# nianticlabs/simplerecon

Measured on AMD Instinct MI355X. Metric: depth frames/sec (640x480, 7 src views, 64 planes), higher is better.
Workload: dtype f32

## Files before the change

include/simplerecon_hip.h:

```cpp
#ifndef SIMPLERECON_HIP_H_
#define SIMPLERECON_HIP_H_

#include <stddef.h>
#include <stdint.h>

#ifdef __cplusplus
extern "C" {
#endif

#define SR_OK 0
#define SR_ERR_INVALID_ARGUMENT 1
#define SR_ERR_UNSUPPORTED 2
#define SR_ERR_WORKSPACE_TOO_SMALL 3
#define SR_ERR_HIP_BASE 1000

enum {
  SR_OPT_MLP_SPLIT = 0, SR_OPT_WINO_SPLIT, SR_OPT_WINO_XCD, SR_OPT_WINO_NT, SR_OPT_WINO_KSPLIT, SR_OPT_CONV_WINO,
  SR_OPT_CONV_TILE, SR_OPT_CONV_KSPLIT, SR_OPT_PW_NT, SR_OPT_PW_KS, SR_OPT_PT_CFG, SR_OPT_PT_KS, SR_OPT_DOT_LDS,
  SR_OPT_DOT_LDS_G, SR_OPT_DOT_LDS_CULL, SR_OPT_DOT_LDS_CAP, SR_OPT_UPSAMPLE_QUAD, SR_OPT_POOL_STREAM,
  SR_OPT_COUNT
};
int sr_option_count(void);
const char* sr_option_name(int id);
int sr_option_id(const char* name);
int sr_option_get(int id, int* value);
int sr_option_set(int id, int value, int* previous );
int sr_option_default(int id, int* value);

int sr_abi_version(void);

const char* sr_target_arch(void);


size_t sr_volume_workspace_bytes(int B, int K, int C, int h, int w);

int sr_volume_prepare(const float* src, const float* K_src, const float* T_src_cur,
                      const float* T_cur_src, int B, int K, int C, int h, int w, void* workspace,
                      size_t workspace_bytes, void* stream);

int sr_dot_volume_sweep(const float* cur, const float* invK_cur, const float* planes, int64_t ps_b,
                        int64_t ps_d, int64_t ps_y, int64_t ps_x, int B, int K, int C, int h, int w,
                        int D, float* out_cv, int64_t cv_sb, int64_t cv_sd, int64_t cv_sp,
                        float* out_lowest, uint8_t* out_mask, void* workspace,
                        size_t workspace_bytes, void* stream);

int sr_conv3x3_wino_io_nhwc_fwd(const void* in, int64_t in_batch_stride, int in_pix_stride, const float* packed_u,
                                const float* bias, const void* residual, int64_t res_batch_stride, int res_pix_stride,
                                void* out, int64_t out_batch_stride, int out_pix_stride, int B, int H, int W, int Cin,
                                int Cout, float leaky_slope, int io_dtype, void* stream);
int sr_pw_conv_io_nhwc_fwd(const void* in, int64_t in_batch_stride, int in_pix_stride, const float* packed_w,
                           const float* bias, const void* residual, int64_t res_batch_stride, int res_pix_stride, void* out,
                           int64_t out_batch_stride, int out_pix_stride, int B, int HW, int Cin, int Cout, float act_code,
                           int io_dtype, void* stream);

size_t sr_pw_conv_tiled_workspace_bytes(int M, int Cin, int Cout);
int sr_pw_conv_tiled_plan(int M, int Cin, int Cout, int can_split, int* cfg, int* ks);
int sr_pw_conv_tiled_nhwc_fwd(const float* in, int in_pix_stride, const float* packed_w, const float* bias,
                              const float* gate, const float* residual, int res_pix_stride, float* out,
                              int out_pix_stride, int M, int HW, int Cin, int Cout, float act_code, void* workspace,
                              size_t workspace_bytes, void* stream);
int sr_pw_conv_supported(int Cin, int Cout);
int sr_pw_conv_plan(int B, int HW, int Cin, int Cout, int* nt, int* ks);
int sr_pw_conv_nhwc_fwd(const float* in, int64_t in_batch_stride, int in_pix_stride, const float* packed_w,
                        const float* bias, const float* gate, const float* residual, int64_t res_batch_stride,
                        int res_pix_stride, float* out, int64_t out_batch_stride, int out_pix_stride, int B, int HW,
                        int Cin, int Cout, float act_code, void* stream);

int sr_backproject_fwd(const float* depth, const float* invK, float* out_points, int B, int h, int w, void* stream);
int sr_project3d_fwd(const float* points, const float* K, const float* T, float* out, int B, int N, float eps,
                     void* stream);
int sr_backproject_bwd(const float* grad_points, const float* invK, float* grad_depth, int B, int h, int w, void* stream);
int sr_project3d_bwd(const float* grad_out, const float* points, const float* K, const float* T, float* grad_points, int B,
// ... 89 lines not shown

int sr_conv3x3_wino4_variant_nhwc_fwd(const float* in, int64_t in_batch_stride, int in_pix_stride, const float* packed_u,
                                      const float* bias, const float* residual, int64_t res_batch_stride,
                                      int res_pix_stride, float* out, int64_t out_batch_stride, int out_pix_stride, int B,
                                      int H, int W, int Cin, int Cout, float leaky_slope, int variant, void* stream);

int sr_wino_splitk_factor(int B, int H, int W, int Cin, int Cout);
size_t sr_wino_splitk_workspace_bytes(int B, int H, int W, int Cin, int Cout);
int sr_conv3x3_wino_splitk_nhwc_fwd(const float* in, int64_t in_batch_stride, int in_pix_stride,
                                    const float* packed_u, const float* bias, const float* residual,
                                    int64_t res_batch_stride, int res_pix_stride, float* out,
                                    int64_t out_batch_stride, int out_pix_stride, int B, int H, int W, int Cin,
                                    int Cout, float leaky_slope, void* workspace, size_t workspace_bytes,
                                    void* stream);

const char* sr_wino_kernel_name(int B, int H, int W, int Cin, int Cout, int aligned_in, int aligned_out);

const char* sr_conv_kernel_name(int B, int H, int W, int Cin, int Cout, int ksize, int stride, int aligned16);

int sr_upsample2x_nhwc_fwd(const float* in, int64_t in_batch_stride, int in_pix_stride, float* out,
                           int64_t out_batch_stride, int out_pix_stride, int B, int H, int W, int C,
                           void* stream);

int sr_exp_fwd(const float* in, float* out, int64_t n, void* stream);


size_t sr_stem_packed_weight_floats(int Cout);
int sr_stem_pack_weights(const float* weight, int Cout, float* packed, void* stream);

int sr_stem7x7_fwd(const float* in, int64_t in_batch_stride, int64_t in_chan_stride, int64_t in_row_stride,
                   int64_t in_col_stride, const float* packed_weight, const float* scale, const float* shift,
                   float leaky_slope, float* out, int64_t out_batch_stride, int out_pix_stride, int B, int H, int W,
                   int Cout, void* stream);

int sr_maxblurpool_nhwc_fwd(const float* in, int64_t in_batch_stride, int in_pix_stride, float* out,
                            int64_t out_batch_stride, int out_pix_stride, int B, int H, int W, int C, void* stream);

size_t sr_instance_norm_workspace_bytes(int B, int H, int W, int C);
int sr_instance_norm_nhwc_fwd(const float* in, int64_t in_batch_stride, int in_pix_stride, float* out,
                              int64_t out_batch_stride, int out_pix_stride, int B, int H, int W, int C, float eps,
                              float leaky_slope, void* workspace, size_t workspace_bytes, void* stream);

int sr_instance_norm_stats_nhwc(const float* in, int64_t in_batch_stride, int in_pix_stride, int B, int H, int W, int C,
                                float eps, float* stats, void* workspace, size_t workspace_bytes, void* stream);

size_t sr_conv1x1_stats_workspace_bytes(int B, int H, int W, int Cout);
int sr_conv1x1_stats_nhwc_fwd(const float* in, int64_t in_batch_stride, int in_pix_stride, const float* weight,
                              const float* bias, float* out, int64_t out_batch_stride, int out_pix_stride, int B, int H,
                              int W, int Cin, int Cout, float eps, float* stats, void* workspace, size_t workspace_bytes,
                              void* stream);

size_t sr_conv3x3_c16_packed_weight_floats(int Cout, int Cin);
int sr_conv3x3_c16_pack_weights(const float* weight, int Cout, int Cin, float* packed, void* stream);
int sr_conv3x3_c16_nhwc_fwd(const float* in, int64_t in_batch_stride, int in_pix_stride, const float* in_stats,
                            float in_leaky_slope, const float* packed_weight, const float* bias, float* out,
                            int64_t out_batch_stride, int out_pix_stride, int B, int H, int W, int Cin, int Cout,
                            int replicate, float leaky_slope, void* stream);

int sr_tsdf_integrate_fwd(void* tsdf_values, void* tsdf_weights, const void* voxel_coords, int X, int Y, int Z,
                          float origin_x, float origin_y, float origin_z, float voxel_size, const void* depth,
                          const uint8_t* depth_mask, const void* K, const void* T, int B, int H, int W,
                          float min_depth, float max_depth, float depth_range, float truncation, float maxW,
                          void* stream);

size_t sr_mesh_count_scratch_bytes(int X, int Y, int Z);
size_t sr_mesh_list_scratch_bytes(int64_t active);
int sr_mesh_count(const void* tsdf_values, int X, int Y, int Z, float level, void* count_scratch,
                  size_t count_scratch_bytes, int64_t* totals, void* stream);
int sr_mesh_emit(const void* tsdf_values, int X, int Y, int Z, float level, float origin_x, float origin_y, float origin_z,
                 float scale, const void* count_scratch, size_t count_scratch_bytes, void* list_scratch,
                 size_t list_scratch_bytes, int64_t active, int64_t num_vertices, int64_t num_faces, float* vertices,
                 float* normals, int* faces, void* stream);

#define SR_PC_FRAME_FLOATS 36
int sr_pc_consistency(const float* depth, const float* frame_consts, int N, int h, int w, int ref_begin, int ref_count,
                      float z_thresh, float* points, int* counts, void* stream);
int sr_pc_voxel_keys(const float* points, int64_t M, double min_x, double min_y, double min_z, double voxel_size,
                     int64_t* keys, void* stream);
int sr_pc_voxel_mean(const float* points, const uint8_t* colors, int64_t M, const int64_t* order,
                     const int64_t* seg_start, int64_t S, float* out_points, uint8_t* out_colors, void* stream);

#define SR_LOSS_MAX_SOURCES 15
size_t sr_normals_workspace_bytes(int B, int h, int w);
int sr_normals_fwd(const float* depth, const float* invK, int B, int h, int w, float* normals, void* scratch,
                   size_t scratch_bytes, void* stream);
int sr_normals_bwd(const float* grad_normals, const float* depth, const float* invK, int B, int h, int w,
                   float* grad_depth, void* scratch, size_t scratch_bytes, void* stream);
size_t sr_normals_loss_workspace_bytes(int B, int h, int w);
int sr_normals_loss_fwd(const float* normals_gt, const float* normals_pred, int B, int h, int w, float* out,
                        void* scratch, size_t scratch_bytes, void* stream);
int sr_normals_loss_bwd(const float* grad_out, const float* stats, const float* normals_gt, const float* normals_pred,
                        int B, int h, int w, float* grad_pred, void* stream);
size_t sr_grad_loss_workspace_bytes(int B, int h, int w);
int sr_grad_loss_fwd(const float* depth_gt, const float* depth_pred, int B, int h, int w, float* out, void* scratch,
                     size_t scratch_bytes, void* stream);
int sr_grad_loss_bwd(const float* grad_out, const float* stats, const float* depth_gt, const float* depth_pred, int B,
                     int h, int w, float* grad_pred, void* scratch, size_t scratch_bytes, void* stream);
size_t sr_mv_loss_workspace_bytes(int B, int K, int h, int w);
int sr_mv_loss_fwd(const float* depth_pred, const float* depth_gt, const float* src_depth, const float* cur_invK,
                   const float* src_K, const float* cur_world_T_cam, const float* src_cam_T_world, int B, int K, int h,
                   int w, float eps, float* out, uint8_t* valid_mask, float* sampled, void* scratch,
                   size_t scratch_bytes, void* stream);
int sr_mv_loss_bwd(const float* grad_out, const float* stats, const float* depth_pred, const float* depth_gt,
                   const float* src_depth, const float* cur_invK, const float* src_K, const float* cur_world_T_cam,
                   const float* src_cam_T_world, int B, int K, int h, int w, float eps, float* grad_pred,
                   void* stream);
// ... 221 lines not shown
```

simplerecon_amd/_lib.py:

```python
import contextlib
import ctypes as C
import os

import torch

_HERE = os.path.dirname(os.path.abspath(__file__))
LIB_PATH = os.environ.get("SR_HIP_LIBRARY") or os.path.join(_HERE, "libsimplerecon_hip.so")
ABI_VERSION = 3

_lib = None

_p = C.c_void_p
_i = C.c_int
_i64 = C.c_int64
_f = C.c_float
_sz = C.c_size_t

SIGNATURES = {
    "sr_abi_version": (_i, []),
    "sr_option_count": (_i, []),
    "sr_option_name": (C.c_char_p, [_i]),
    "sr_option_id": (_i, [C.c_char_p]),
    "sr_option_get": (_i, [_i, C.POINTER(C.c_int)]),
    "sr_option_set": (_i, [_i, _i, C.POINTER(C.c_int)]),
# ... 65 lines not shown
    "sr_norm_stats_nhwc": (_i, [_p, _i64, _i, _i, _i, _i, _i, _p, _p, _p, _sz, _p]),
    "sr_norm_act_fwd_nhwc": (_i, [_p, _i64, _i, _p, _p, _f, _p, _p, _f, _i, _p, _i64, _i, _i, _i, _i, _p]),
    "sr_norm_act_bwd_nhwc": (_i, [_p, _i64, _i, _p, _i64, _i, _p, _p, _f, _p, _p, _f, _i, _i, _p, _i64, _i, _p, _p,
                                  _i, _i, _i, _p, _sz, _p]),
    "sr_rowsum_nhwc": (_i, [_p, _i64, _i, _p, _i64, _i, _i, _i, _i, _f, _p, _p, _sz, _p]),
    "sr_maxblurpool_bwd_workspace_bytes": (_sz, [_i, _i, _i, _i]),
    "sr_maxblurpool_bwd_nhwc": (_i, [_p, _i64, _i, _p, _i64, _i, _p, _i64, _i, _i, _i, _i, _i, _p, _sz, _p]),
    "sr_replicate_pad_nhwc_fwd": (_i, [_p, _i64, _i, _p, _i, _i, _i, _i, _i, _p]),
    "sr_replicate_pad_nhwc_bwd": (_i, [_p, _p, _i, _i, _i, _i, _i, _p]),
    "sr_im2col7x7s2_nhwc": (_i, [_p, _i64, _i64, _i64, _i64, _p, _i, _i, _i, _i, _p]),
    "sr_dwconv3x3_bwd_workspace_bytes": (_sz, [_i, _i, _i, _i]),
    "sr_dwconv3x3_bwd_nhwc": (_i, [_p, _i64, _i, _p, _i64, _i, _p, _p, _p, _i, _i, _i, _i, _i, _i, _i, _i, _i, _p, _sz,
                                   _p]),
    "sr_scale_bwd_nhwc": (_i, [_p, _i64, _i, _p, _p, _f, _p, _i, _i, _i, _p]),
    "sr_small_linear_fwd": (_i, [_p, _p, _p, _p, _p, _i, _i, _i, _f, _p]),
    "sr_small_linear_bwd": (_i, [_p, _p, _p, _p, _p, _p, _p, _i, _i, _i, _f, _p]),
    "sr_act_in_bwd": (_i, [_p, _p, _p, _i64, _f, _p]),
    "sr_add_act_fwd": (_i, [_p, _p, _p, _p, _i64, _f, _p]),
    "sr_conv_wgrad_padded_workspace_bytes": (_sz, [_i, _i, _i, _i, _i, _i]),
    "sr_conv_wgrad_padded_nhwc": (_i, [_p, _i64, _i, _p, _i64, _i, _p, _i, _i, _i, _i, _i, _i, _i, _i, _i, _i, _i, _p,
                                       _sz, _p]),
    "sr_conv_splitk_workspace_bytes": (_sz, [_i, _i, _i, _i, _i, _i, _i]),
    "sr_conv2d_splitk_nhwc_fwd": (_i, [_p, _i64, _i, _p, _p, _p, _i64, _i, _p, _i64, _i, _i, _i, _i, _i, _i, _i, _i,
                                       _f, _p, _sz, _p]),
    "sr_wino_packed_weight_floats": (_sz, [_i, _i]),
    "sr_wino_pack_weights": (_i, [_p, _i, _i, _p, _p]),
    "sr_conv_prefers_wino": (_i, [_i, _i, _i, _i, _i, _i, _i]),
    "sr_wino_splitk_factor": (_i, [_i, _i, _i, _i, _i]),
    "sr_wino_splitk_workspace_bytes": (_sz, [_i, _i, _i, _i, _i]),
    "sr_conv3x3_wino_splitk_nhwc_fwd": (_i, [_p, _i64, _i, _p, _p, _p, _i64, _i, _p, _i64, _i, _i, _i, _i, _i, _i, _f,
                                             _p, _sz, _p]),
    "sr_wino_kernel_name": (C.c_char_p, [_i, _i, _i, _i, _i, _i, _i]),
    "sr_conv3x3_wino_nhwc_fwd": (_i, [_p, _i64, _i, _p, _p, _p, _i64, _i, _p, _i64, _i, _i, _i, _i, _i, _i, _f, _p]),
    "sr_wino4_packed_weight_floats": (_sz, [_i, _i]),
    "sr_wino4_pack_weights": (_i, [_p, _i, _i, _p, _p]),
    "sr_conv_prefers_wino4": (_i, [_i, _i, _i, _i, _i, _i]),
    "sr_conv3x3_wino4_nhwc_fwd": (_i, [_p, _i64, _i, _p, _p, _p, _i64, _i, _p, _i64, _i, _i, _i, _i, _i, _i, _f, _p]),
    "sr_conv3x3_wino4_variant_nhwc_fwd": (_i, [_p, _i64, _i, _p, _p, _p, _i64, _i, _p, _i64, _i, _i, _i, _i, _i, _i, _f, _i,
                                               _p]),
    "sr_conv_kernel_name": (C.c_char_p, [_i, _i, _i, _i, _i, _i, _i, _i]),
    "sr_upsample2x_nhwc_fwd": (_i, [_p, _i64, _i, _p, _i64, _i, _i, _i, _i, _i, _p]),
    "sr_exp_fwd": (_i, [_p, _p, _i64, _p]),
    "sr_stem_packed_weight_floats": (_sz, [_i]),
    "sr_stem_pack_weights": (_i, [_p, _i, _p, _p]),
    "sr_stem7x7_fwd": (_i, [_p, _i64, _i64, _i64, _i64, _p, _p, _p, _f, _p, _i64, _i, _i, _i, _i, _i, _p]),
    "sr_maxblurpool_nhwc_fwd": (_i, [_p, _i64, _i, _p, _i64, _i, _i, _i, _i, _i, _p]),
    "sr_instance_norm_workspace_bytes": (_sz, [_i, _i, _i, _i]),
    "sr_instance_norm_nhwc_fwd": (_i, [_p, _i64, _i, _p, _i64, _i, _i, _i, _i, _i, _f, _f, _p, _sz, _p]),
    "sr_instance_norm_stats_nhwc": (_i, [_p, _i64, _i, _i, _i, _i, _i, _f, _p, _p, _sz, _p]),
    "sr_conv1x1_stats_workspace_bytes": (_sz, [_i, _i, _i, _i]),
    "sr_conv1x1_stats_nhwc_fwd": (_i, [_p, _i64, _i, _p, _p, _p, _i64, _i, _i, _i, _i, _i, _i, _f, _p, _p, _sz, _p]),
    "sr_conv3x3_c16_packed_weight_floats": (_sz, [_i, _i]),
    "sr_conv3x3_c16_pack_weights": (_i, [_p, _i, _i, _p, _p]),
    "sr_conv3x3_c16_nhwc_fwd": (_i, [_p, _i64, _i, _p, _f, _p, _p, _p, _i64, _i, _i, _i, _i, _i, _i, _i, _f, _p]),
    "sr_tsdf_integrate_fwd": (_i, [_p, _p, _p, _i, _i, _i, _f, _f, _f, _f, _p, _p, _p, _p, _i, _i, _i,
                                   _f, _f, _f, _f, _f, _p]),
    "sr_mesh_count_scratch_bytes": (_sz, [_i, _i, _i]),
    "sr_mesh_list_scratch_bytes": (_sz, [_i64]),
    "sr_mesh_count": (_i, [_p, _i, _i, _i, _f, _p, _sz, _p, _p]),
    "sr_mesh_emit": (_i, [_p, _i, _i, _i, _f, _f, _f, _f, _f, _p, _sz, _p, _sz, _i64, _i64, _i64, _p, _p, _p, _p]),
    "sr_pc_consistency": (_i, [_p, _p, _i, _i, _i, _i, _i, _f, _p, _p, _p]),
    "sr_pc_voxel_keys": (_i, [_p, _i64, C.c_double, C.c_double, C.c_double, C.c_double, _p, _p]),
    "sr_pc_voxel_mean": (_i, [_p, _p, _i64, _p, _p, _i64, _p, _p, _p]),
    "sr_normals_workspace_bytes": (_sz, [_i, _i, _i]),
    "sr_normals_fwd": (_i, [_p, _p, _i, _i, _i, _p, _p, _sz, _p]),
    "sr_normals_bwd": (_i, [_p, _p, _p, _i, _i, _i, _p, _p, _sz, _p]),
    "sr_normals_loss_workspace_bytes": (_sz, [_i, _i, _i]),
    "sr_normals_loss_fwd": (_i, [_p, _p, _i, _i, _i, _p, _p, _sz, _p]),
    "sr_normals_loss_bwd": (_i, [_p, _p, _p, _p, _i, _i, _i, _p, _p]),
    "sr_grad_loss_workspace_bytes": (_sz, [_i, _i, _i]),
    "sr_grad_loss_fwd": (_i, [_p, _p, _i, _i, _i, _p, _p, _sz, _p]),
    "sr_grad_loss_bwd": (_i, [_p, _p, _p, _p, _i, _i, _i, _p, _p, _sz, _p]),
    "sr_mv_loss_workspace_bytes": (_sz, [_i, _i, _i, _i]),
    "sr_mv_loss_fwd": (_i, [_p, _p, _p, _p, _p, _p, _p, _i, _i, _i, _i, _f, _p, _p, _p, _p, _sz, _p]),
    "sr_mv_loss_bwd": (_i, [_p, _p, _p, _p, _p, _p, _p, _p, _p, _i, _i, _i, _i, _f, _p, _p]),
    "sr_depth_terms_workspace_bytes": (_sz, [_i, _i, _i]),
    "sr_depth_terms_fwd": (_i, [_p, _p, _p, _p, _p, _i, _i, _p, _i, _i, _p, _i, _i, _i, _i, _i, _f, _i, _p, _p, _sz,
                                _p]),
    "sr_depth_terms_bwd": (_i, [_p, _p, _p, _p, _p, _p, _p, _i, _i, _p, _i, _i, _p, _i, _i, _i, _i, _i, _f, _i, _p, _p,
                                _p, _p, _p, _p]),
    "sr_depth_metrics_workspace_bytes": (_sz, [_i, _i, _i]),
    "sr_depth_metrics": (_i, [_p, _p, _p, _f, _i, _i, _i, _i, _i, _i, _i, _p, _p, _p, _p, _sz, _p]),
    "sr_depth_metrics_gather": (_i, [_p, _i, _i, _i, _i, _i, _i, _p, _p]),
    "sr_nn_grid_plan": (_i, [_i64, _p, _i64, _p, _p, _p]),
    "sr_nn_keys": (_i, [_p, _i64, C.c_double, C.c_double, C.c_double, C.c_double, _i, _i, _i, _p, _p]),
    "sr_nn_build": (_i, [_p, _i64, _p, _p, _i64, _p, _p, _p]),
    "sr_nn_query": (_i, [_p, _i64, _p, _p, _i64, _p, _i64, C.c_double, C.c_double, C.c_double, C.c_double, _i, _i, _i,
                         _p, _p, _p, _p]),
    "sr_sample_surface_workspace_bytes": (_sz, [_i64]),
    "sr_sample_surface_cdf": (_i, [_p, _i64, _p, _i64, _p, _p, _sz, _p]),
    "sr_sample_surface": (_i, [_p, _i64, _p, _i64, _p, _i64, C.c_uint64, _p, _p, _p]),
    "sr_mesh_metrics_workspace_bytes": (_sz, [_i64, _i64]),
    "sr_mesh_metrics": (_i, [_p, _i64, _p, _i64, _f, _p, _p, _sz, _p]),
    "sr_stsdf_touch": (_i, [_p, _i, _i, _i, _p, C.c_double, C.c_double, _p, _p]),
    "sr_stsdf_block_masks": (_i, [_p, _p, _i64, _i64, _p, _p]),
    "sr_stsdf_integrate": (_i, [_p, _i64, _p, _p, _p, _i64, _p, _p, _p, _i, _i, _i, _f, _f, _p]),
    "sr_stsdf_mesh_count": (_i, [_p, _i64, _p, _p, _i64, _p, _p]),
    "sr_stsdf_mesh_emit": (_i, [_p, _i64, _p, _p, _i64, _f, _p, _i64, _i64, _p, _p, _p, _p, _p]),
    "sr_raster_small": (_i, [_p, _i64, _p, _i64, _p, _p, _i, _i, _i, _f, _f, _i, _p, _p, _p]),
    "sr_raster_large_setup": (_i, [_p, _i64, _p, _i64, _p, _p, _i, _i, _i, _f, _f, _i, _i64, _p, _p, _p, _p]),
    "sr_raster_large": (_i, [_p, _p, _i64, _i64, _p, _i, _i, _i, _f, _f, _p, _p]),
    "sr_raster_resolve": (_i, [_p, _i64, _p, _p, _p]),
    "sr_raster_visibility_mask": (_i, [_p, _i, _i64, _i64, _p, _p]),
    "sr_raster_visibility_count": (_i, [_p, _i64, _p, _i, _p, _p]),
    "sr_frames_resize_fits_lds": (_i, [_i, _i, _i, _i]),
    "sr_frames_resize": (_i, [_p, _i, _i, _i, _i, _p, _i, _p, _i, _i, _p, _p, _i, _i, _i, _i, _p, _p]),
# ... 192 lines not shown
```

simplerecon_amd/csrc/sr_matching.hip:

```cpp
#include "sr_common.h"

typedef float v16f __attribute__((ext_vector_type(16)));
#define SR_MFMA(a, b, c) __builtin_amdgcn_mfma_f32_32x32x2f32((a), (b), (c), 0, 0, 0)

#define SR_STEM_T 16
#define SR_STEM_PR 37
#define SR_STEM_PW 37
#define SR_STEM_STEPS 74
#define SR_STEM_WFLOATS (SR_STEM_STEPS * 128)
#define SR_STEM_PFLOATS (3 * SR_STEM_PR * SR_STEM_PW)

struct SrStemParams {
  const float* in; int64_t sb, sc, sy, sx;
  const float* wp;
  const float* scale; const float* shift;
  float slope;
  float* out; int64_t out_sb; int out_sp;
  int H, W, Ho, Wo, tiles_x, tiles_y, total;
};

__global__ void sr_stem_pack_kernel(const float* __restrict__ w , float* __restrict__ packed) {
  for (int idx = blockIdx.x * blockDim.x + threadIdx.x; idx < SR_STEM_WFLOATS; idx += gridDim.x * blockDim.x) {
    const int step = idx >> 7, r = idx & 127;
    const int half = r >> 6, col = (r & 63) >> 1, nt = r & 1;
    const int tap = 2 * step + half;
    const int co = nt * 32 + col;
    packed[idx] = tap < 147 ? w[co * 147 + tap] : 0.f;
  }
}

__host__ __device__ constexpr int sr_stem_tap_offset(int k) {
  return k >= 147 ? 0 : ((k / 49) * SR_STEM_PR + (k % 49) / 7) * SR_STEM_PW + (k % 7);
}

__global__ __launch_bounds__(256, 2) void sr_stem_kernel(SrStemParams p) {
  __shared__ __attribute__((aligned(16))) float wl[SR_STEM_WFLOATS];
  __shared__ float patch[SR_STEM_PFLOATS];
  const int lane = threadIdx.x & 63, wave = threadIdx.x >> 6;
  const int i = lane & 31, half = lane >> 5;

  for (int e = threadIdx.x; e < SR_STEM_WFLOATS / 4; e += 256)
    reinterpret_cast<float4*>(wl)[e] = reinterpret_cast<const float4*>(p.wp)[e];

  int abase[2];
#pragma unroll
  for (int m = 0; m < 2; ++m) abase[m] = (2 * (4 * wave + 2 * m + (i >> 4))) * SR_STEM_PW + 2 * (i & 15);
  const float2* wl2 = reinterpret_cast<const float2*>(wl) + half * 32 + i;

  float sc[2], sh[2];
#pragma unroll
  for (int n = 0; n < 2; ++n) {
    sc[n] = p.scale ? p.scale[n * 32 + i] : 1.f;
    sh[n] = p.shift ? p.shift[n * 32 + i] : 0.f;
// ... 613 lines not shown
#pragma unroll
      for (int r = 0; r < 4; ++r) acc[m][r] = 0.f;

    __syncthreads();
    stage_load(0);
    stage_store(0, tiles[0]);
    __syncthreads();
    for (int slab = 0; slab < slabs; ++slab) {
      const float* tl = tiles[slab & 1];
      const bool more = slab + 1 < slabs;
      if (more) stage_load(slab + 1);
      const float4* ws = wl + (size_t)slab * 9 * 2 * 64;
      float4 wA = ws[0], wB = ws[64];
#pragma unroll
      for (int step = 0; step < 18; ++step) {
        const int tap = step >> 1, g = step & 1, ky = tap / 3, kx = tap % 3;
        const float4 w = wA;
        wA = wB;
        if (step + 2 < 18) wB = ws[(step + 2) * 64];
        float4 a[2];
#pragma unroll
        for (int m = 0; m < 2; ++m)
          a[m] = *reinterpret_cast<const float4*>(&tl[((2 * wave + m + ky) * SR_T16_HW + li + kx) * SR_T16_ROW + 16 * g + 4 * lk]);
#pragma unroll
        for (int m = 0; m < 2; ++m) {
          acc[m] = __builtin_amdgcn_mfma_f32_16x16x4f32(a[m].x, w.x, acc[m], 0, 0, 0);
          acc[m] = __builtin_amdgcn_mfma_f32_16x16x4f32(a[m].y, w.y, acc[m], 0, 0, 0);
          acc[m] = __builtin_amdgcn_mfma_f32_16x16x4f32(a[m].z, w.z, acc[m], 0, 0, 0);
          acc[m] = __builtin_amdgcn_mfma_f32_16x16x4f32(a[m].w, w.w, acc[m], 0, 0, 0);
        }
      }
      if (more) stage_store(slab + 1, tiles[(slab + 1) & 1]);
      __syncthreads();
    }

    float* __restrict__ ob = p.out + (int64_t)b * p.out_sb;
    const float bv = (p.bias && li < p.Cout) ? p.bias[li] : 0.f;
#pragma unroll
    for (int m = 0; m < 2; ++m) {
      const int oy = oy0 + 2 * wave + m;
#pragma unroll
      for (int r = 0; r < 4; ++r) {
        const int ox = ox0 + 4 * lk + r;
        if (oy < p.H && ox < p.W && li < p.Cout) {
          float v = acc[m][r] + bv;
          if (p.out_slope >= 0.f) v = v >= 0.f ? v : v * p.out_slope;
          ob[((int64_t)oy * p.W + ox) * p.out_sp + li] = v;
        }
      }
    }
  }
}


static int sr_cus() { return sr_device_cus(); }

extern "C" size_t sr_conv3x3_c16_packed_weight_floats(int Cout, int Cin) {
  if (Cout <= 0 || Cout > 16 || Cin <= 0 || (Cin % 32)) return 0;
  return (size_t)(Cin / 32) * 9 * 2 * 64 * 4;
}

extern "C" int sr_conv3x3_c16_pack_weights(const float* weight, int Cout, int Cin, float* packed, void* stream_) {
  if (!weight || !packed) return SR_ERR_INVALID_ARGUMENT;
  if (Cout <= 0 || Cout > 16 || Cin <= 0 || (Cin % 32)) return SR_ERR_UNSUPPORTED;
  hipLaunchKernelGGL(sr_t16_pack_kernel, dim3(64), dim3(256), 0, (hipStream_t)stream_, weight, packed, Cout, Cin);
  return sr_hip_rc(hipGetLastError());
}

extern "C" int sr_conv3x3_c16_nhwc_fwd(const float* in, int64_t in_batch_stride, int in_pix_stride,
                                       const float* in_stats, float in_leaky_slope, const float* packed_weight,
                                       const float* bias, float* out, int64_t out_batch_stride, int out_pix_stride,
                                       int B, int H, int W, int Cin, int Cout, int replicate, float leaky_slope,
                                       void* stream_) {
  if (B < 0 || H <= 0 || W <= 0 || Cin <= 0 || Cout <= 0) return SR_ERR_INVALID_ARGUMENT;
  if (B == 0) return SR_OK;
  if (!in || !packed_weight || !out) return SR_ERR_INVALID_ARGUMENT;
  if (Cout > 16 || (Cin % 32) || (in_pix_stride % 4) || (in_batch_stride % 4) || ((uintptr_t)in & 15) ||
      (in_stats && ((uintptr_t)in_stats & 15)))
    return SR_ERR_UNSUPPORTED;
  SrT16Params p;
  p.in = in; p.in_sb = in_batch_stride; p.in_sp = in_pix_stride;
  p.stats = in_stats; p.in_slope = in_leaky_slope;
  p.wp = packed_weight; p.bias = bias;
  p.out = out; p.out_sb = out_batch_stride; p.out_sp = out_pix_stride;
  p.H = H; p.W = W; p.Cin = Cin; p.Cout = Cout; p.replicate = replicate;
  p.tiles_x = (W + 15) / 16; p.tiles_y = (H + 7) / 8;
  p.total = p.tiles_x * p.tiles_y * B;
  p.out_slope = leaky_slope;
  int blocks = 3 * sr_cus();
  if (blocks > p.total) blocks = p.total;
  const bool norm = in_stats != nullptr, act = in_leaky_slope >= 0.f;
  if (norm && act) hipLaunchKernelGGL((sr_t16_kernel<true, true>), dim3(blocks), dim3(256), 0, (hipStream_t)stream_, p);
  else if (norm) hipLaunchKernelGGL((sr_t16_kernel<true, false>), dim3(blocks), dim3(256), 0, (hipStream_t)stream_, p);
  else if (act) hipLaunchKernelGGL((sr_t16_kernel<false, true>), dim3(blocks), dim3(256), 0, (hipStream_t)stream_, p);
  else hipLaunchKernelGGL((sr_t16_kernel<false, false>), dim3(blocks), dim3(256), 0, (hipStream_t)stream_, p);
  return sr_hip_rc(hipGetLastError());
}

extern "C" size_t sr_stem_packed_weight_floats(int Cout) { return Cout == 64 ? (size_t)SR_STEM_WFLOATS : 0; }

extern "C" int sr_stem_pack_weights(const float* weight, int Cout, float* packed, void* stream_) {
  if (!weight || !packed) return SR_ERR_INVALID_ARGUMENT;
  if (Cout != 64) return SR_ERR_UNSUPPORTED;
  hipLaunchKernelGGL(sr_stem_pack_kernel, dim3(42), dim3(256), 0, (hipStream_t)stream_, weight, packed);
  return sr_hip_rc(hipGetLastError());
}

extern "C" int sr_stem7x7_fwd(const float* in, int64_t in_batch_stride, int64_t in_chan_stride, int64_t in_row_stride,
                              int64_t in_col_stride, const float* packed_weight, const float* scale,
                              const float* shift, float leaky_slope, float* out, int64_t out_batch_stride,
                              int out_pix_stride, int B, int H, int W, int Cout, void* stream_) {
  if (B < 0 || H <= 0 || W <= 0) return SR_ERR_INVALID_ARGUMENT;
  if (Cout != 64) return SR_ERR_UNSUPPORTED;
  if (B == 0) return SR_OK;
  if (!in || !packed_weight || !out) return SR_ERR_INVALID_ARGUMENT;
  SrStemParams p;
  p.in = in; p.sb = in_batch_stride; p.sc = in_chan_stride; p.sy = in_row_stride; p.sx = in_col_stride;
  p.wp = packed_weight; p.scale = scale; p.shift = shift; p.slope = leaky_slope;
  p.out = out; p.out_sb = out_batch_stride; p.out_sp = out_pix_stride;
  p.H = H; p.W = W;
  p.Ho = (H + 6 - 7) / 2 + 1; p.Wo = (W + 6 - 7) / 2 + 1;
  p.tiles_x = (p.Wo + SR_STEM_T - 1) / SR_STEM_T; p.tiles_y = (p.Ho + SR_STEM_T - 1) / SR_STEM_T;
  p.total = p.tiles_x * p.tiles_y * B;
  int blocks = 2 * sr_cus();
  if (blocks > p.total) blocks = p.total;
  hipLaunchKernelGGL(sr_stem_kernel, dim3(blocks), dim3(256), 0, (hipStream_t)stream_, p);
  return sr_hip_rc(hipGetLastError());
}

extern "C" int sr_maxblurpool_nhwc_fwd(const float* in, int64_t in_batch_stride, int in_pix_stride, float* out,
                                       int64_t out_batch_stride, int out_pix_stride, int B, int H, int W, int C,
                                       void* stream_) {
  if (B < 0 || H < 4 || W < 4 || C <= 0) return SR_ERR_INVALID_ARGUMENT;
  if (B == 0) return SR_OK;
  if (!in || !out) return SR_ERR_INVALID_ARGUMENT;
  if ((C % 4) || (in_pix_stride % 4) || (out_pix_stride % 4) || (in_batch_stride % 4) || (out_batch_stride % 4) ||
      ((uintptr_t)in & 15) || ((uintptr_t)out & 15))
    return SR_ERR_UNSUPPORTED;
  const int Ho = (H - 2) / 2 + 1, Wo = (W - 2) / 2 + 1;
  if (sr_opt(SR_OPT_POOL_STREAM) && H >= 16 && W >= 16 && B <= 65535) {
    SrPoolStreamParams p;
    p.in = in; p.in_sb = in_batch_stride; p.in_sp = in_pix_stride;
    p.out = out; p.out_sb = out_batch_stride; p.out_sp = out_pix_stride;
    p.H = H; p.W = W; p.Ho = Ho; p.Wo = Wo; p.C4 = C / 4;
    p.oy_lo = 1; p.oy_hi = (H - 4) / 2; p.ox_lo = 1; p.ox_hi = (W - 4) / 2;
    const int rows = p.oy_hi - p.oy_lo + 1, cols = p.ox_hi - p.ox_lo + 1;
    p.col_blocks = (cols + 1) / 2;
    p.col_groups = (int)(((int64_t)p.col_blocks * p.C4 + 255) / 256);
// ... 133 lines not shown
```

simplerecon_amd/csrc/sr_options.hip:

```cpp
#include <atomic>
#include <mutex>
#include <stdlib.h>
#include <string.h>

#include "sr_common.h"

namespace {

struct OptDef { const char* name; int dflt; int kind; };
const OptDef kDefs[SR_OPT_COUNT] = {
    {"SR_MLP_SPLIT", 0, 1},       {"SR_WINO_SPLIT", 0, 1},     {"SR_WINO_XCD", 1, 0},        {"SR_WINO_NT", 0, 0},
    {"SR_WINO_KSPLIT", 0, 0},     {"SR_CONV_WINO", 1, 0},      {"SR_CONV_TILE", 0, 0},       {"SR_CONV_KSPLIT", 1, 0},
    {"SR_PW_NT", 0, 0},           {"SR_PW_KS", 0, 0},          {"SR_PT_CFG", -1, 0},         {"SR_PT_KS", 0, 0},
    {"SR_DOT_LDS", 1, 0},         {"SR_DOT_LDS_G", 0, 0},      {"SR_DOT_LDS_CULL", 1, 0},    {"SR_DOT_LDS_CAP", 634, 0},
    {"SR_UPSAMPLE_QUAD", 1, 0},   {"SR_POOL_STREAM", 1, 0},
};
std::atomic<int> g_val[SR_OPT_COUNT];
std::once_flag g_once;

int parse(const OptDef& d, const char* e) {
  if (d.kind == 1) {
    if (!e || !*e || !strcmp(e, "0") || !strcmp(e, "off") || !strcmp(e, "fp32")) return 0;
    if (!strcmp(e, "bf16")) return 1;
    if (!strcmp(e, "f16") || !strcmp(e, "fp16")) return 2;
    return -1;
  }
  return (e && *e) ? atoi(e) : d.dflt;
}

void init() {
  for (int i = 0; i < SR_OPT_COUNT; ++i) {
    const char* e = getenv(kDefs[i].name);
    g_val[i].store(e ? parse(kDefs[i], e) : kDefs[i].dflt, std::memory_order_relaxed);
  }
}

}

int sr_opt(int id) {
  std::call_once(g_once, init);
  return g_val[id].load(std::memory_order_relaxed);
}

extern "C" int sr_option_count(void) { return SR_OPT_COUNT; }

extern "C" const char* sr_option_name(int id) { return (id >= 0 && id < SR_OPT_COUNT) ? kDefs[id].name : nullptr; }

extern "C" int sr_option_id(const char* name) {
  if (!name) return -1;
  for (int i = 0; i < SR_OPT_COUNT; ++i)
    if (!strcmp(kDefs[i].name, name)) return i;
  return -1;
}

extern "C" int sr_option_get(int id, int* value) {
  if (id < 0 || id >= SR_OPT_COUNT || !value) return SR_ERR_INVALID_ARGUMENT;
  *value = sr_opt(id);
  return SR_OK;
}

extern "C" int sr_option_set(int id, int value, int* previous) {
  if (id < 0 || id >= SR_OPT_COUNT) return SR_ERR_INVALID_ARGUMENT;
  std::call_once(g_once, init);
  const int old = g_val[id].exchange(value, std::memory_order_relaxed);
  if (previous) *previous = old;
  return SR_OK;
}

// ... 19 lines not shown
```

simplerecon_amd/ops.py:

```python
import ctypes as C
import contextlib
import os
import weakref

import torch
from torch import nn

from . import _lib

PROFILE = None

_PACKED = weakref.WeakKeyDictionary()
_NO_ENTRIES = {}


def _cached(mod, tag, key, build, *args):
    e = _PACKED.get(mod, _NO_ENTRIES).get(tag)
    if e is not None and e[0] == key:
        if e[2] is not None:
            _await_pack(e)
        return e[1]
    payload = build(*args)
    fence = None
    if _lib.cuda_available() and not _lib.capturing():
# ... 548 lines not shown
    isb, isp = _strides(x)
    _lib.call("sr_instance_norm_stats_nhwc", x.device, x, isb, isp, b, h, w, c, eps, stats, ws, ws.numel() * 4)
    return stats


def conv1x1_stats(x, conv: nn.Conv2d, eps=1e-5):
    _lib.refuse_autograd(x, conv.weight)
    x = as_nhwc(x, "conv input")
    b, ci, h, w = x.shape
    co = conv.out_channels
    if conv.kernel_size != (1, 1) or conv.stride != (1, 1) or tuple(conv.padding) != (0, 0) or conv.groups != 1 \
            or (ci, co) != (64, 128) or ci != conv.in_channels:
        raise _lib.HipLibraryError(f"conv1x1_stats needs Conv2d(64, 128, 1), got {conv} for {ci} channels")
    out = empty_nhwc(b, co, h, w, x.device)
    stats = torch.empty((b, 2, co), dtype=torch.float32, device=x.device)
    if b == 0:
        return out, stats
    lib = _lib.lib()
    ws = _workspace(x.device, "c1s", lib.sr_conv1x1_stats_workspace_bytes(b, h, w, co))
    weight = conv.weight.detach().reshape(co, ci).contiguous()
    bias = conv.bias.detach() if conv.bias is not None else None
    isb, isp = _strides(x)
    osb, osp = _strides(out)
    record = lambda: ("sr_conv1x1_stats_kernel", 2.0 * b * h * w * co * ci, (b, ci, h, w, co, 1, 1),
                      2.0 * b * ((h * w + 63) // 64) * 64 * co * ci)
    rc = _timed(x.device, record, lib.sr_conv1x1_stats_nhwc_fwd, _lib.ptr(x), isb, isp, _lib.ptr(weight), _lib.ptr(bias),
                _lib.ptr(out), osb, osp, b, h, w, ci, co, eps, _lib.ptr(stats), _lib.ptr(ws), ws.numel() * 4,
                _lib.stream_ptr(x.device))
    _lib.check(rc, "sr_conv1x1_stats_nhwc_fwd")
    return out, stats


def _pack_c16(conv):
    return _pack("conv3x3_c16", conv.weight.detach().contiguous()), (conv.bias.detach() if conv.bias is not None else None)


def conv3x3_c16(x, conv: nn.Conv2d, in_stats=None, in_leaky=None, leaky=None):
    _lib.refuse_autograd(x, conv.weight)
    x = as_nhwc(x, "conv input")
    b, ci, h, w = x.shape
    co = conv.out_channels
    if conv.kernel_size != (3, 3) or conv.stride != (1, 1) or tuple(conv.padding) != (1, 1) or conv.groups != 1 \
            or conv.dilation != (1, 1) or conv.padding_mode not in ("zeros", "replicate") or co > 16 or ci % 32 \
            or ci != conv.in_channels:
        raise _lib.HipLibraryError(f"conv3x3_c16 needs Conv2d(32k, <=16, 3, padding=1), got {conv} for {ci} channels")
    wp, bias = _cached(conv, "c16", _state_key(conv, None), _pack_c16, conv)
    if in_stats is not None and (tuple(in_stats.shape) != (b, 2, ci) or not in_stats.is_contiguous()):
        raise ValueError(f"in_stats must be a contiguous [{b}, 2, {ci}] tensor")
    out = empty_nhwc(b, co, h, w, x.device)
    if b == 0:
        return out
    isb, isp = _strides(x)
    osb, osp = _strides(out)
    record = lambda: ("sr_t16_kernel", 2.0 * b * h * w * co * ci * 9, (b, ci, h, w, co, 3, 1),
                      2.0 * b * ((h + 7) // 8) * ((w + 15) // 16) * 128 * 16 * ci * 9)
    rc = _timed(x.device, record, _lib.lib().sr_conv3x3_c16_nhwc_fwd, _lib.ptr(x), isb, isp, _lib.ptr(in_stats),
                -1.0 if in_leaky is None else float(in_leaky), _lib.ptr(wp), _lib.ptr(bias), _lib.ptr(out), osb,
                osp, b, h, w, ci, co, int(conv.padding_mode == "replicate"),
                -1.0 if leaky is None else float(leaky), _lib.stream_ptr(x.device))
    _lib.check(rc, "sr_conv3x3_c16_nhwc_fwd")
    return out



def _pack_dw(conv, bn):
    w, bias = _effective_weight(conv, bn)
    return w.reshape(conv.in_channels, 9).t().contiguous(), (bias.contiguous() if bias is not None else None)


def packed_dw_weight(conv: nn.Conv2d, bn=None):
    _lib.require_device_f32("depthwise conv weight", conv.weight)
    c = conv.in_channels
    if conv.kernel_size != (3, 3) or conv.groups != c or conv.out_channels != c or conv.dilation != (1, 1) \
            or conv.padding_mode != "zeros":
        raise _lib.HipLibraryError(f"unsupported depthwise Conv2d configuration for the HIP path: {conv}")
    return _cached(conv, "dw", _state_key(conv, bn), _pack_dw, conv, bn)


def dwconv3x3(x, conv: nn.Conv2d, bn=None, leaky=None, act=None, tf_same=False, want_pool=False, pads=None):
    _lib.refuse_autograd(x, conv.weight)
    x = as_nhwc(x, "depthwise conv input")
    b, c, h, w = x.shape
    if c != conv.in_channels:
        raise ValueError(f"depthwise conv expects {conv.in_channels} channels, got {c}")
    s = conv.stride[0]
    if conv.stride[0] != conv.stride[1] or s not in (1, 2):
        raise _lib.HipLibraryError(f"unsupported stride {conv.stride}")
    if pads is None and not tf_same and tuple(conv.padding) != (1, 1):
        raise _lib.HipLibraryError(f"unsupported padding {conv.padding}")
    if pads is None:
        pads = tf_same_pads(h, w, 3, s) if tf_same else (1, 1, 1, 1)
    ho, wo = (h + pads[0] + pads[2] - 3) // s + 1, (w + pads[1] + pads[3] - 3) // s + 1
    w9c, bias = packed_dw_weight(conv, bn)
    lib = _lib.lib()
    out = empty_nhwc(b, c, ho, wo, x.device)
    bands = lib.sr_dwconv3x3_pool_bands(ho)
    pool = torch.empty((b, bands, c), dtype=torch.float32, device=x.device) if want_pool else None
    if b > 0:
        isb, isp = _strides(x)
        osb, osp = _strides(out)
        _lib.call("sr_dwconv3x3_nhwc_fwd", x.device, x, isb, isp, w9c, bias, out, osb, osp, pool, b, h, w, c, s, *pads,
                  _act_code(leaky, act))
    return (out, pool) if want_pool else out


def se_gate(pool_partial, pixels, conv_reduce: nn.Conv2d, conv_expand: nn.Conv2d):
    _lib.require_device_f32("pool partial sums", pool_partial)
    b, bands, c = pool_partial.shape
# ... 121 lines not shown
```

Before: 315.0.

## Add Winograd F(2x2,3x3) path for small-Cout 3x3 conv via MFMA

Adds a Winograd F(2,3) variant of the Cout<=16 3x3 convolution kernel. It packs transformed weights alongside the direct ones, transforms input tiles of 16x16 outputs in LDS, and runs 16 MFMA 16x16x4 GEMMs per slab, which cuts multiply count versus direct 9-tap convolution. It is enabled by default when the tile count exceeds three blocks per CU. In exchange it uses a larger halo tile and more packed-weight memory, with some Winograd numerical error.

```diff
diff --git a/include/simplerecon_hip.h b/include/simplerecon_hip.h
--- a/include/simplerecon_hip.h
+++ b/include/simplerecon_hip.h
@@ -18,6 +18,7 @@
   SR_OPT_MLP_SPLIT = 0, SR_OPT_WINO_SPLIT, SR_OPT_WINO_XCD, SR_OPT_WINO_NT, SR_OPT_WINO_KSPLIT, SR_OPT_CONV_WINO,
   SR_OPT_CONV_TILE, SR_OPT_CONV_KSPLIT, SR_OPT_PW_NT, SR_OPT_PW_KS, SR_OPT_PT_CFG, SR_OPT_PT_KS, SR_OPT_DOT_LDS,
   SR_OPT_DOT_LDS_G, SR_OPT_DOT_LDS_CULL, SR_OPT_DOT_LDS_CAP, SR_OPT_UPSAMPLE_QUAD, SR_OPT_POOL_STREAM,
+  SR_OPT_T16_WINO,
   SR_OPT_COUNT
 };
 int sr_option_count(void);
@@ -213,6 +214,7 @@
 
 size_t sr_conv3x3_c16_packed_weight_floats(int Cout, int Cin);
 int sr_conv3x3_c16_pack_weights(const float* weight, int Cout, int Cin, float* packed, void* stream);
+const char* sr_conv3x3_c16_kernel_name(int B, int H, int W, int Cin, int Cout);
 int sr_conv3x3_c16_nhwc_fwd(const float* in, int64_t in_batch_stride, int in_pix_stride, const float* in_stats,
                             float in_leaky_slope, const float* packed_weight, const float* bias, float* out,
                             int64_t out_batch_stride, int out_pix_stride, int B, int H, int W, int Cin, int Cout,
diff --git a/simplerecon_amd/_lib.py b/simplerecon_amd/_lib.py
--- a/simplerecon_amd/_lib.py
+++ b/simplerecon_amd/_lib.py
@@ -141,6 +141,7 @@
     "sr_conv1x1_stats_nhwc_fwd": (_i, [_p, _i64, _i, _p, _p, _p, _i64, _i, _i, _i, _i, _i, _i, _f, _p, _p, _sz, _p]),
     "sr_conv3x3_c16_packed_weight_floats": (_sz, [_i, _i]),
     "sr_conv3x3_c16_pack_weights": (_i, [_p, _i, _i, _p, _p]),
+    "sr_conv3x3_c16_kernel_name": (C.c_char_p, [_i, _i, _i, _i, _i]),
     "sr_conv3x3_c16_nhwc_fwd": (_i, [_p, _i64, _i, _p, _f, _p, _p, _p, _i64, _i, _i, _i, _i, _i, _i, _i, _f, _p]),
     "sr_tsdf_integrate_fwd": (_i, [_p, _p, _p, _i, _i, _i, _f, _f, _f, _f, _p, _p, _p, _p, _i, _i, _i,
                                    _f, _f, _f, _f, _f, _p]),
diff --git a/simplerecon_amd/csrc/sr_matching.hip b/simplerecon_amd/csrc/sr_matching.hip
--- a/simplerecon_amd/csrc/sr_matching.hip
+++ b/simplerecon_amd/csrc/sr_matching.hip
@@ -1,4 +1,7 @@
+#include <type_traits>
+
 #include "sr_common.h"
+#include "sr_wino.h"
 
 typedef float v16f __attribute__((ext_vector_type(16)));
 #define SR_MFMA(a, b, c) __builtin_amdgcn_mfma_f32_32x32x2f32((a), (b), (c), 0, 0, 0)
@@ -718,19 +721,265 @@
   }
 }
 
+#define SR_T16W_ROW 20
+#define SR_T16W_HALO 18
+#define SR_T16W_TILE (SR_T16W_HALO * SR_T16W_HALO * SR_T16W_ROW)
+#define SR_T16W_STAGE 6
+#define SR_T16W_NW 4
+
+__global__ void sr_t16_wino_pack_kernel(const float* __restrict__ w , float* __restrict__ packed, int Cout,
+                                        int Cin) {
+  const float G[4][3] = {{1.f, 0.f, 0.f}, {0.5f, 0.5f, 0.5f}, {0.5f, -0.5f, 0.5f}, {0.f, 0.f, 1.f}};
+  const int total = (Cin / 16) * 16 * 64 * 4;
+  for (int e = blockIdx.x * blockDim.x + threadIdx.x; e < total; e += gridDim.x * blockDim.x) {
+    const int s = e & 3, lane = (e >> 2) & 63, f = (e >> 8) & 15, slab = e >> 12;
+    const int co = lane & 15, ci = 16 * slab + 4 * (lane >> 4) + s, fr = f >> 2, fc = f & 3;
+    float u = 0.f;
+    if (co < Cout) {
+      const float* g = w + ((size_t)co * Cin + ci) * 9;
+      for (int kx = 0; kx < 3; ++kx) {
+        float t = 0.f;
+        for (int ky = 0; ky < 3; ++ky) t += G[fr][ky] * g[ky * 3 + kx];
+        u += t * G[fc][kx];
+      }
+    }
+    packed[e] = u;
+  }
+}
+
+template <bool NORM, bool IN_ACT>
+__global__ __launch_bounds__(256, 3) void sr_t16_wino_kernel(SrT16Params p) {
+  __shared__ __attribute__((aligned(16))) float tiles[2][SR_T16W_TILE];
+  const int tid = threadIdx.x, lane = tid & 63, wave = tid >> 6;
+  const int li = lane & 15, lk = lane >> 4;
+  const int slabs = p.Cin >> 4;
+  const int cq = tid & 3;
+  const int G = (int)gridDim.x;
+  const int per_tile = p.tiles_x * p.tiles_y;
+  const float4* wl = reinterpret_cast<const float4*>(p.wp) + lane;
+  const int wsteps = slabs * 16;
+  const int a_base = ((4 * wave + 2 * (li >> 3)) * SR_T16W_HALO + 2 * (li & 7)) * SR_T16W_ROW + 4 * lk;
+
+  auto tile_of = [&](int work) {
+    if ((G & 7) == 0) {
+      const int r0 = work / G * G;
+      if (r0 + G <= p.total) { const int bb = work - r0; return r0 + (bb & 7) * (G >> 3) + (bb >> 3); }
+    }
+    return work;
+  };
+
+  float neg1s = -1.0f;
+  asm volatile("" : "+s"(neg1s));
+  const wn_f2 neg1 = {neg1s, neg1s};
+  auto sub4 = [&](const float4 x, const float4 y) {
+    const wn_f2 lo = __builtin_elementwise_fma(neg1, wn_f2{y.x, y.y}, wn_f2{x.x, x.y});
+    const wn_f2 hi = __builtin_elementwise_fma(neg1, wn_f2{y.z, y.w}, wn_f2{x.z, x.w});
+    return make_float4(lo.x, lo.y, hi.x, hi.y);
+  };
+
+  unsigned offs[SR_T16W_STAGE];
+  unsigned pad = 0;
+  const char* in_b = reinterpret_cast<const char*>(p.in);
+  const float* st = nullptr;
+  auto aim = [&](int work) __attribute__((always_inline)) {
+    const int tile = tile_of(work);
+    const int b = tile / per_tile, t2 = tile - b * per_tile, ty = t2 / p.tiles_x, tx = t2 - ty * p.tiles_x;
+    in_b = reinterpret_cast<const char*>(p.in + (int64_t)b * p.in_sb);
+    if (NORM) st = p.stats + (int64_t)b * 2 * p.Cin;
+    pad = 0;
+#pragma unroll
+    for (int it = 0; it < SR_T16W_STAGE; ++it) {
+      const int e = tid + it * 256, px = e >> 2;
+      const int hy = px / SR_T16W_HALO, hx = px - hy * SR_T16W_HALO;
+      int iy = 16 * ty - 1 + hy, ix = 16 * tx - 1 + hx;
+      if (p.replicate) { iy = min(max(iy, 0), p.H - 1); ix = min(max(ix, 0), p.W - 1); }
+      const bool ok = (px < SR_T16W_HALO * SR_T16W_HALO) & (iy >= 0) & (iy < p.H) & (ix >= 0) & (ix < p.W);
+      offs[it] = ok ? (unsigned)((iy * p.W + ix) * p.in_sp + 4 * cq) * 4u : 0u;
+      pad |= ok ? 0u : 1u << it;
+    }
+  };
+  float4 stg[SR_T16W_STAGE];
+  auto stage_load = [&](int slab) __attribute__((always_inline)) {
+    const char* src = in_b + 64 * slab;
+#pragma unroll
+    for (int it = 0; it < SR_T16W_STAGE; ++it) stg[it] = *reinterpret_cast<const float4*>(src + offs[it]);
+  };
+  const bool fast_leaky = IN_ACT && p.in_slope <= 1.0f;
+  const wn_f2 slope2 = {p.in_slope, p.in_slope};
+  auto stage_store_as = [&](int slab, float* tl, auto fast_tag, auto zpad_tag) __attribute__((always_inline)) {
+    constexpr bool FAST = decltype(fast_tag)::value, ZPAD = decltype(zpad_tag)::value;
+    wn_f2 nm[2] = {{0.f, 0.f}, {0.f, 0.f}}, r[2] = {{1.f, 1.f}, {1.f, 1.f}};
+    if (NORM) {
+      const float4 m4 = *reinterpret_cast<const float4*>(st + 16 * slab + 4 * cq);
+      const float4 r4 = *reinterpret_cast<const float4*>(st + p.Cin + 16 * slab + 4 * cq);
+      nm[0] = wn_f2{-m4.x, -m4.y}; nm[1] = wn_f2{-m4.z, -m4.w};
+      r[0] = wn_f2{r4.x, r4.y}; r[1] = wn_f2{r4.z, r4.w};
+    }
+#pragma unroll
+    for (int it = 0; it < SR_T16W_STAGE; ++it) {
+      const int e = tid + it * 256, px = e >> 2;
+      if (px < SR_T16W_HALO * SR_T16W_HALO) {
+        wn_f2 v[2] = {{stg[it].x, stg[it].y}, {stg[it].z, stg[it].w}};
+#pragma unroll
+        for (int h = 0; h < 2; ++h) {
+          if (NORM) v[h] = (v[h] + nm[h]) * r[h];
+          if (IN_ACT) {
+            if (FAST) {
+              const wn_f2 sv = v[h] * slope2;
+              v[h] = wn_f2{fmaxf(v[h].x, sv.x), fmaxf(v[h].y, sv.y)};
+            } else {
+              v[h].x = v[h].x >= 0.f ? v[h].x : v[h].x * p.in_slope;
+              v[h].y = v[h].y >= 0.f ? v[h].y : v[h].y * p.in_slope;
+            }
+          }
+        }
+        float4 o = make_float4(v[0].x, v[0].y, v[1].x, v[1].y);
+        if (ZPAD && ((pad >> it) & 1u)) o = make_float4(0.f, 0.f, 0.f, 0.f);
+        *reinterpret_cast<float4*>(&tl[px * SR_T16W_ROW + 4 * cq]) = o;
+      }
+    }
+  };
+  auto stage_store = [&](int slab, float* tl) __attribute__((always_inline)) {
+    if (p.replicate) {
+      if (fast_leaky) stage_store_as(slab, tl, std::true_type{}, std::false_type{});
+      else stage_store_as(slab, tl, std::false_type{}, std::false_type{});
+    } else {
+      if (fast_leaky) stage_store_as(slab, tl, std::true_type{}, std::true_type{});
+      else stage_store_as(slab, tl, std::false_type{}, std::true_type{});
+    }
+  };
+
+  int work = blockIdx.x;
+  if (work >= p.total) return;
+  aim(work);
+  stage_load(0);
+  stage_store(0, tiles[0]);
+  float4 wr[SR_T16W_NW];
+#pragma unroll
+  for (int j = 0; j < SR_T16W_NW; ++j) wr[j] = wl[j * 64];
+  int wnext = SR_T16W_NW;
+  __syncthreads();
+
+  int par = 0;
+  for (; work < p.total; work += G) {
+    const int tile = tile_of(work);
+    const int b = tile / per_tile, t2 = tile - b * per_tile, ty = t2 / p.tiles_x, tx = t2 - ty * p.tiles_x;
+    f32x4 acc[16];
+    auto slab_body = [&](int slab, auto first) __attribute__((always_inline)) {
+      const float* tl = tiles[par] + a_base;
+      int nslab = slab + 1;
+      bool more = nslab < slabs;
+      if (!more && work + G < p.total) { aim(work + G); nslab = 0; more = true; }
+      if (more) stage_load(nslab);
+
+      float4 d1[4], d2[4], t[4];
+#pragma unroll
+      for (int c = 0; c < 4; ++c) {
+        d1[c] = *reinterpret_cast<const float4*>(&tl[(1 * SR_T16W_HALO + c) * SR_T16W_ROW]);
+        d2[c] = *reinterpret_cast<const float4*>(&tl[(2 * SR_T16W_HALO + c) * SR_T16W_ROW]);
+      }
+#pragma unroll
+      for (int fr = 0; fr < 4; ++fr) {
+#pragma unroll
+        for (int c = 0; c < 4; ++c) {
+          if (fr == 0) t[c] = sub4(*reinterpret_cast<const float4*>(&tl[c * SR_T16W_ROW]), d2[c]);
+          else if (fr == 1) t[c] = f4add(d1[c], d2[c]);
+          else if (fr == 2) t[c] = sub4(d2[c], d1[c]);
+          else t[c] = sub4(d1[c], *reinterpret_cast<const float4*>(&tl[(3 * SR_T16W_HALO + c) * SR_T16W_ROW]));
+        }
+        const float4 v[4] = {sub4(t[0], t[2]), f4add(t[1], t[2]), sub4(t[2], t[1]), sub4(t[1], t[3])};
+        const float vs[4][4] = {{v[0].x, v[0].y, v[0].z, v[0].w}, {v[1].x, v[1].y, v[1].z, v[1].w},
+                                {v[2].x, v[2].y, v[2].z, v[2].w}, {v[3].x, v[3].y, v[3].z, v[3].w}};
+        float ws[4][4];
+#pragma unroll
+        for (int fc = 0; fc < 4; ++fc) {
+          ws[fc][0] = wr[fc].x; ws[fc][1] = wr[fc].y; ws[fc][2] = wr[fc].z; ws[fc][3] = wr[fc].w;
+        }
+#pragma unroll
+        for (int j = 0; j < 16; ++j) {
+          const int k = j & 3, fc = j >> 2;
+          const int f = 4 * fr + fc;
+          if (k == 0 && decltype(first)::value) {
+            const f32x4 z = {0.f, 0.f, 0.f, 0.f};
+            acc[f] = __builtin_amdgcn_mfma_f32_16x16x4f32(vs[fc][k], ws[fc][k], z, 0, 0, 0);
+          } else {
+            acc[f] = __builtin_amdgcn_mfma_f32_16x16x4f32(vs[fc][k], ws[fc][k], acc[f], 0, 0, 0);
+          }
+        }
+#pragma unroll
+        for (int fc = 0; fc < 4; ++fc) {
+          wr[fc] = wl[(size_t)wnext * 64];
+          wnext = wnext + 1 == wsteps ? 0 : wnext + 1;
+        }
+      }
+      if (more) stage_store(nslab, tiles[par ^ 1]);
+      __syncthreads();
+      par ^= 1;
+    };
+    slab_body(0, std::true_type{});
+    for (int slab = 1; slab < slabs; ++slab) slab_body(slab, std::false_type{});
+
+    float* __restrict__ ob = p.out + (int64_t)b * p.out_sb;
+    const float bv = (p.bias && li < p.Cout) ? p.bias[li] : 0.f;
+    const int oyb = 16 * ty + 4 * wave + 2 * (lk >> 1), oxb = 16 * tx + 8 * (lk & 1);
+#pragma unroll
+    for (int r = 0; r < 4; ++r) {
+      float y[2][2];
+#pragma unroll
+      for (int dx = 0; dx < 2; ++dx) {
+        float c[4];
+#pragma unroll
+        for (int fr = 0; fr < 4; ++fr)
+          c[fr] = dx == 0 ? acc[4 * fr][r] + acc[4 * fr + 1][r] + acc[4 * fr + 2][r]
+                          : acc[4 * fr + 1][r] - acc[4 * fr + 2][r] - acc[4 * fr + 3][r];
+        y[0][dx] = c[0] + c[1] + c[2];
+        y[1][dx] = c[1] - c[2] - c[3];
+      }
+#pragma unroll
+      for (int dy = 0; dy < 2; ++dy)
+#pragma unroll
+        for (int dx = 0; dx < 2; ++dx) {
+          const int oy = oyb + dy, ox = oxb + 2 * r + dx;
+          if (oy < p.H && ox < p.W && li < p.Cout) {
+            float v = y[dy][dx] + bv;
+            if (p.out_slope >= 0.f) v = v >= 0.f ? v : v * p.out_slope;
+            ob[((int64_t)oy * p.W + ox) * p.out_sp + li] = v;
+          }
+        }
+    }
+  }
+}
+
 
 static int sr_cus() { return sr_device_cus(); }
+
+static size_t sr_t16_direct_floats(int Cin) { return (size_t)(Cin / 32) * 9 * 2 * 64 * 4; }
+static size_t sr_t16_wino_floats(int Cin) { return (size_t)(Cin / 16) * 16 * 64 * 4; }
+
+static bool sr_t16_use_wino(int B, int H, int W, int Cin) {
+  const int mode = sr_opt(SR_OPT_T16_WINO);
+  if (mode == 0 || (Cin % 16)) return false;
+  if (mode == 2) return true;
+  return (int64_t)B * ((H + 7) / 8) * ((W + 15) / 16) > 3 * (int64_t)sr_cus();
+}
 
 extern "C" size_t sr_conv3x3_c16_packed_weight_floats(int Cout, int Cin) {
   if (Cout <= 0 || Cout > 16 || Cin <= 0 || (Cin % 32)) return 0;
-  return (size_t)(Cin / 32) * 9 * 2 * 64 * 4;
+  return sr_t16_direct_floats(Cin) + sr_t16_wino_floats(Cin);
 }
 
 extern "C" int sr_conv3x3_c16_pack_weights(const float* weight, int Cout, int Cin, float* packed, void* stream_) {
   if (!weight || !packed) return SR_ERR_INVALID_ARGUMENT;
   if (Cout <= 0 || Cout > 16 || Cin <= 0 || (Cin % 32)) return SR_ERR_UNSUPPORTED;
   hipLaunchKernelGGL(sr_t16_pack_kernel, dim3(64), dim3(256), 0, (hipStream_t)stream_, weight, packed, Cout, Cin);
+  hipLaunchKernelGGL(sr_t16_wino_pack_kernel, dim3(64), dim3(256), 0, (hipStream_t)stream_, weight,
+                     packed + sr_t16_direct_floats(Cin), Cout, Cin);
   return sr_hip_rc(hipGetLastError());
+}
+
+extern "C" const char* sr_conv3x3_c16_kernel_name(int B, int H, int W, int Cin, int Cout) {
+  (void)Cout;
+  return sr_t16_use_wino(B, H, W, Cin) ? "sr_t16_wino_kernel" : "sr_t16_kernel";
 }
 
 extern "C" int sr_conv3x3_c16_nhwc_fwd(const float* in, int64_t in_batch_stride, int in_pix_stride,
@@ -744,22 +993,32 @@
   if (Cout > 16 || (Cin % 32) || (in_pix_stride % 4) || (in_batch_stride % 4) || ((uintptr_t)in & 15) ||
       (in_stats && ((uintptr_t)in_stats & 15)))
     return SR_ERR_UNSUPPORTED;
+  const bool wino = sr_t16_use_wino(B, H, W, Cin) && (int64_t)H * W * in_pix_stride < ((int64_t)1 << 30);
   SrT16Params p;
   p.in = in; p.in_sb = in_batch_stride; p.in_sp = in_pix_stride;
   p.stats = in_stats; p.in_slope = in_leaky_slope;
-  p.wp = packed_weight; p.bias = bias;
+  p.wp = wino ? packed_weight + sr_t16_direct_floats(Cin) : packed_weight; p.bias = bias;
   p.out = out; p.out_sb = out_batch_stride; p.out_sp = out_pix_stride;
   p.H = H; p.W = W; p.Cin = Cin; p.Cout = Cout; p.replicate = replicate;
-  p.tiles_x = (W + 15) / 16; p.tiles_y = (H + 7) / 8;
+  p.tiles_x = (W + 15) / 16; p.tiles_y = wino ? (H + 15) / 16 : (H + 7) / 8;
   p.total = p.tiles_x * p.tiles_y * B;
   p.out_slope = leaky_slope;
   int blocks = 3 * sr_cus();
   if (blocks > p.total) blocks = p.total;
   const bool norm = in_stats != nullptr, act = in_leaky_slope >= 0.f;
-  if (norm && act) hipLaunchKernelGGL((sr_t16_kernel<true, true>), dim3(blocks), dim3(256), 0, (hipStream_t)stream_, p);
-  else if (norm) hipLaunchKernelGGL((sr_t16_kernel<true, false>), dim3(blocks), dim3(256), 0, (hipStream_t)stream_, p);
-  else if (act) hipLaunchKernelGGL((sr_t16_kernel<false, true>), dim3(blocks), dim3(256), 0, (hipStream_t)stream_, p);
-  else hipLaunchKernelGGL((sr_t16_kernel<false, false>), dim3(blocks), dim3(256), 0, (hipStream_t)stream_, p);
+  const dim3 grid(blocks), wg(256);
+  hipStream_t stream = (hipStream_t)stream_;
+  if (wino) {
+    if (norm && act) hipLaunchKernelGGL((sr_t16_wino_kernel<true, true>), grid, wg, 0, stream, p);
+    else if (norm) hipLaunchKernelGGL((sr_t16_wino_kernel<true, false>), grid, wg, 0, stream, p);
+    else if (act) hipLaunchKernelGGL((sr_t16_wino_kernel<false, true>), grid, wg, 0, stream, p);
+    else hipLaunchKernelGGL((sr_t16_wino_kernel<false, false>), grid, wg, 0, stream, p);
+  } else {
+    if (norm && act) hipLaunchKernelGGL((sr_t16_kernel<true, true>), grid, wg, 0, stream, p);
+    else if (norm) hipLaunchKernelGGL((sr_t16_kernel<true, false>), grid, wg, 0, stream, p);
+    else if (act) hipLaunchKernelGGL((sr_t16_kernel<false, true>), grid, wg, 0, stream, p);
+    else hipLaunchKernelGGL((sr_t16_kernel<false, false>), grid, wg, 0, stream, p);
+  }
   return sr_hip_rc(hipGetLastError());
 }
 
diff --git a/simplerecon_amd/csrc/sr_options.hip b/simplerecon_amd/csrc/sr_options.hip
--- a/simplerecon_amd/csrc/sr_options.hip
+++ b/simplerecon_amd/csrc/sr_options.hip
@@ -13,7 +13,7 @@
     {"SR_WINO_KSPLIT", 0, 0},     {"SR_CONV_WINO", 1, 0},      {"SR_CONV_TILE", 0, 0},       {"SR_CONV_KSPLIT", 1, 0},
     {"SR_PW_NT", 0, 0},           {"SR_PW_KS", 0, 0},          {"SR_PT_CFG", -1, 0},         {"SR_PT_KS", 0, 0},
     {"SR_DOT_LDS", 1, 0},         {"SR_DOT_LDS_G", 0, 0},      {"SR_DOT_LDS_CULL", 1, 0},    {"SR_DOT_LDS_CAP", 634, 0},
-    {"SR_UPSAMPLE_QUAD", 1, 0},   {"SR_POOL_STREAM", 1, 0},
+    {"SR_UPSAMPLE_QUAD", 1, 0},   {"SR_POOL_STREAM", 1, 0},     {"SR_T16_WINO", 1, 0},
 };
 std::atomic<int> g_val[SR_OPT_COUNT];
 std::once_flag g_once;
diff --git a/simplerecon_amd/ops.py b/simplerecon_amd/ops.py
--- a/simplerecon_amd/ops.py
+++ b/simplerecon_amd/ops.py
@@ -624,8 +624,11 @@
         return out
     isb, isp = _strides(x)
     osb, osp = _strides(out)
-    record = lambda: ("sr_t16_kernel", 2.0 * b * h * w * co * ci * 9, (b, ci, h, w, co, 3, 1),
-                      2.0 * b * ((h + 7) // 8) * ((w + 15) // 16) * 128 * 16 * ci * 9)
+    def record():
+        name = _lib.lib().sr_conv3x3_c16_kernel_name(b, h, w, ci, co).decode()
+        tiles = b * ((h + 15) // 16) * ((w + 15) // 16) * 64 if "wino" in name else 0
+        executed = 2.0 * tiles * 16 * 16 * ci if tiles else 2.0 * b * ((h + 7) // 8) * ((w + 15) // 16) * 128 * 16 * ci * 9
+        return name, 2.0 * b * h * w * co * ci * 9, (b, ci, h, w, co, 3, 1), executed
     rc = _timed(x.device, record, _lib.lib().sr_conv3x3_c16_nhwc_fwd, _lib.ptr(x), isb, isp, _lib.ptr(in_stats),
                 -1.0 if in_leaky is None else float(in_leaky), _lib.ptr(wp), _lib.ptr(bias), _lib.ptr(out), osb,
                 osp, b, h, w, ci, co, int(conv.padding_mode == "replicate"),
```

Result: no change. 316.5, median of 6 (+0.5%).
